# alpc91/SGRL

Hardware: AMD Instinct MI355X
Metric: env-steps/sec (whole node) + SET-actor fwd us/step, 3d_walker mix @8192 envs/GPU (higher is better)
Workload: dtype f64 (dynamics) / f32 (SET actor, obs); 1 GPU; 3D_Walker++ 8 variants x 1024 envs per GPU (config 3), random U(-1,1) actions, auto-reset, SET actor forward on every step, random-init weights; envs_per_gpu=8192, obs_max_len=287, action_max_len=21, replay_gather=none (single rank)

## Files before the change

include/sgrl.h:

```cpp
#ifndef SGRL_H
#define SGRL_H

#include <stdint.h>

#ifdef __cplusplus
extern "C" {
#endif

typedef struct sgrl_engine sgrl_engine;

enum {
  SGRL_OK = 0,
  SGRL_ERR_ARG = -1,
  SGRL_ERR_MODEL = -2,
  SGRL_ERR_HIP = -3,
  SGRL_ERR_LIMIT = -4
};

int sgrl_engine_create(int n_morph, const int32_t* const* ib, const int32_t* ib_len, const double* const* fb,
                       const int32_t* fb_len, const int32_t* morph_count, int obs_max_len, int action_max_len,
                       uint64_t seed, uint32_t env_id_base, int max_episode_steps, sgrl_engine** out);
void sgrl_engine_destroy(sgrl_engine* e);

int sgrl_num_envs(const sgrl_engine* e);
// ... 10 lines not shown
int sgrl_step(sgrl_engine* e, const float* actions, float* obs, float* reward, uint8_t* done, float* dist,
              uint8_t* truncated, double* obs64, double* reward64, int auto_reset, void* stream);

int sgrl_get_records(sgrl_engine* e, double* rec, int32_t* cnt);
int sgrl_set_records(sgrl_engine* e, const double* rec, const int32_t* cnt);
int sgrl_refresh(sgrl_engine* e, float* obs, double* obs64, void* stream);

int sgrl_time_steps(sgrl_engine* e, const float* actions, float* obs, float* reward, uint8_t* done, int reps,
                    void* stream, float* ms_out);

int sgrl_pack_transitions(const float* obs, int ld_obs, const float* action, int ld_act, const float* next_obs, int ld_next,
                          const float* reward, const float* done_f32, const uint8_t* done_u8, const uint8_t* store,
                          const int64_t* morph_id, float* block, int n_env, int obs_len, int act_len, void* stream);

int sgrl_round_record(const float* reward, const uint8_t* done, uint8_t* done_list, int64_t* ep_steps, float* ep_reward, float* reward_buf,
                      uint8_t* store, float* done_bool, int32_t* all_done, int n_env, int max_episode_steps, void* stream);

int sgrl_round_record_all(const float* reward, const uint8_t* done, uint8_t* done_list, int64_t* ep_steps, float* ep_reward, float* reward_buf,
                          int64_t* cur_steps, uint8_t* store, float* done_bool, int32_t* all_done, int32_t* was_complete, int n_env,
                          int max_episode_steps, void* stream);

typedef struct sgrl_ring {
  float* obs; float* action; float* next_obs; float* reward; float* done;
  int32_t obs_dim, act_dim;
} sgrl_ring;
int sgrl_ingest_rows(const float* block, int n_rows, int obs_len, int act_len, const int64_t* slot, const sgrl_ring* rings,
                     int n_rings, void* stream);
int64_t sgrl_ingest_ws_words(int n_rows);
int sgrl_ingest_block(const float* block, int n_rows, int obs_len, int act_len, const sgrl_ring* rings, int n_rings, int64_t* pos,
                      const int64_t* cap, int64_t* pending, int64_t* slot_ws, void* stream);

#define SGRL_DEBUG_CHOL_LD 352
int sgrl_debug_chol_solve(int flags, const int32_t* n, const double* C, const double* rhs, double* C_out, double* x_out, int32_t* ok);

const char* sgrl_last_error(void);
const char* sgrl_version(void);

#ifdef __cplusplus
}
#endif
#endif
```

sgrl_amd/_lib.py:

```python
import ctypes
import os
import subprocess

_HERE = os.path.dirname(os.path.abspath(__file__))
LIB_PATH = os.environ.get("SGRL_HIP_LIB", os.path.join(_HERE, "libsgrl_hip.so"))
CSRC = os.path.join(_HERE, "csrc")
SOURCES = ["engine.hip", "set_actor.hip", "train_gemm.hip", "render.hip", "swat_actor.hip", "smp_actor.hip", "replay_sample.hip", "eval_record.hip", "explore_actions.hip", "scene.hip", "mlp_actor.hip", "mlp_train.hip", "mlp_optim.hip", "mlp_batch.hip", "smp_train.hip", "td3_loss.hip", "dropout.hip"]

_lib = None

_i32p = ctypes.POINTER(ctypes.c_int32)
_f64p = ctypes.POINTER(ctypes.c_double)


class SgrlError(RuntimeError):
    pass


HDR_DIM_FIELDS = (1, 2, 3, 4, 5, 6, 7, 8, 9, 16, 18)
LIGHT_NV = 12
ITAB_GLOBAL = set(x for x in os.environ.get("SGRL_BUILD_ITAB_GLOBAL", "humanoid").split(",") if x and x != "none")
PAIR_NV = {"walker": 15, "hopper": 15}


# ... 118 lines not shown
    L.sgrl_time_steps.argtypes = [vp, vp, vp, vp, vp, ctypes.c_int, vp, ctypes.POINTER(ctypes.c_float)]
    ci = ctypes.c_int
    L.sgrl_pack_transitions.argtypes = [vp, ci, vp, ci, vp, ci, vp, vp, vp, vp, vp, vp, ci, ci, ci, vp]
    L.sgrl_ingest_rows.argtypes = [vp, ci, ci, ci, vp, vp, ci, vp]
    L.sgrl_ingest_block.argtypes = [vp, ci, ci, ci, vp, ci, vp, vp, vp, vp, vp]
    L.sgrl_reset_where.argtypes = [vp, vp, vp, vp, vp]
    L.sgrl_round_record.argtypes = [vp, vp, vp, vp, vp, vp, vp, vp, vp, ci, ci, vp]
    L.sgrl_round_record_all.argtypes = [vp, vp, vp, vp, vp, vp, vp, vp, vp, vp, vp, ci, ci, vp]
    L.sgrl_ingest_ws_words.argtypes = [ci]
    L.sgrl_ingest_ws_words.restype = ctypes.c_int64
    _lib = L
    return L


EXPLORE_GAUSS, EXPLORE_UNIFORM = 0, 1


def bind_explore(L):
    if getattr(L, "_explore_bound", False):
        return L
    vp, ci, cf = ctypes.c_void_p, ctypes.c_int, ctypes.c_float
    L.sgrl_explore_actions.argtypes = [vp, ci, vp, ci, vp, ci, ci, ctypes.c_int64, ctypes.c_uint64, ctypes.c_uint64, ci, cf, cf, cf, vp]
    L.sgrl_explore_actions.restype = ci
    L.sgrl_explore_actions_launches.argtypes = []
    L.sgrl_explore_actions_launches.restype = ci
    L.sgrl_explore_last_error.argtypes = []
    L.sgrl_explore_last_error.restype = ctypes.c_char_p
    L._explore_bound = True
    return L


EXPORTS = ["sgrl_engine_create", "sgrl_engine_destroy", "sgrl_num_envs", "sgrl_record_stride", "sgrl_lds_bytes", "sgrl_launch_groups", "sgrl_fixed_dim_groups", "sgrl_paired_envs",
           "sgrl_reset", "sgrl_reset_where", "sgrl_step", "sgrl_get_records", "sgrl_set_records", "sgrl_refresh", "sgrl_time_steps", "sgrl_pack_transitions", "sgrl_round_record", "sgrl_round_record_all", "sgrl_ingest_rows", "sgrl_ingest_block", "sgrl_ingest_ws_words",
           "sgrl_debug_chol_solve", "sgrl_last_error", "sgrl_version"]


def check(rc, what):
    if rc != 0:
        raise SgrlError("%s failed (%d): %s" % (what, rc, lib().sgrl_last_error().decode()))
```

sgrl_amd/csrc/engine.hip:

```cpp
#include <hip/hip_runtime.h>

#include <algorithm>
#include <cmath>
#include <cstdio>
#include <cstdlib>
#include <cstring>
#include <string>
#include <vector>

#include "engine_kernel.h"
#include "stream_pick.h"

namespace {

thread_local std::string g_err;

int fail(int code, const std::string& msg) {
  g_err = msg;
  return code;
}
#define HIP_TRY(expr)                                                                              \
  do {                                                                                             \
    hipError_t _e = (expr);                                                                        \
    if (_e != hipSuccess)                                                                          \
// ... 1 lines not shown
  } while (0)

using namespace sgrl_engine_dev;

__global__ __launch_bounds__(64) __attribute__((amdgpu_waves_per_eu(2, 2))) void k_env_step(BatchArgs a, StepOut out) {
  env_step_wave<DimsAny, sgrl::HipWave>(a, out, __builtin_amdgcn_readfirstlane(a.block_env[blockIdx.x]));
}

constexpr int kLightNv = 15;
constexpr int kLightPerCu = 12;
__global__ __launch_bounds__(64) __attribute__((amdgpu_waves_per_eu(3, 3))) void k_env_step_light(BatchArgs a, StepOut out) {
  env_step_wave<DimsAny, sgrl::HipWaveT<kLightNv>>(a, out, __builtin_amdgcn_readfirstlane(a.block_env[blockIdx.x]));
}

__global__ __launch_bounds__(64) void k_env_reset(BatchArgs a, StepOut out) {
  const int env = __builtin_amdgcn_readfirstlane(a.block_env[blockIdx.x]);
  if (out.done && !__builtin_amdgcn_readfirstlane((int)out.done[env])) return;
  SgrlModelView m; sgrl::Layout o; double* S; int32_t* I;
  setup<DimsAny>(a, env, &m, &o, &S, &I);
  sgrl::HipWave w;
  const sgrl::StepIO io = make_io(a, out, env);
  sgrl::env_reset(w, m, o, S, I, io, true);
}

__global__ __launch_bounds__(64) void k_env_refresh(BatchArgs a, StepOut out) {
  const int env = __builtin_amdgcn_readfirstlane(a.block_env[blockIdx.x]);
  SgrlModelView m; sgrl::Layout o; double* S; int32_t* I;
  setup<DimsAny>(a, env, &m, &o, &S, &I);
  sgrl::HipWave w;
  const sgrl::StepIO io = make_io(a, out, env);
  sgrl::env_refresh(w, m, o, S, I, io);
}

template <class Wv>
__device__ __forceinline__ void debug_chol_solve(Wv& w, int n, double* C, double* x, double* wv, bool inverse, int32_t* ok) {
  bool done;
  if (!inverse) {
    done = w.chol_solve_packed(n, C, x, sgrl::kMinVal);
  } else {
    done = w.chol_inv_packed(n, C, sgrl::kMinVal);
    if (done) {
      w.lanes(n, [&](int i) {
        double z = 0;
        for (int c = 0; c <= i; c++) z += C[i * (i + 1) / 2 + c] * x[c];
        wv[i] = z;
      });
      w.lanes(n, [&](int k) {
        double s = 0;
        for (int i = k; i < n; i++) s += C[i * (i + 1) / 2 + k] * wv[i];
        x[k] = s;
      });
    }
  }
  if (w.lane == 0) *ok = done ? 1 : 0;
}
__global__ __launch_bounds__(64) void k_debug_chol_solve(int flags, const int32_t* n, const double* C, const double* rhs, double* C_out,
                                                         double* x_out, int32_t* ok) {
  constexpr int LD = SGRL_DEBUG_CHOL_LD;
  __shared__ double sC[2 * LD], sx[64], swv[64];
  const int t = threadIdx.x;
  for (int i = t; i < 2 * LD; i += 64) sC[i] = C[i];
  sx[t] = rhs[t];
  swv[t] = 0.0;
  __syncthreads();
  if (flags & 1) {
    sgrl::HalfWaveT<15, sgrl::HipHalfPrim<sgrl::DimsAny>> w;
    const int h = w.half;
    debug_chol_solve(w, n[h], sC + h * LD, sx + h * 32, swv + h * 32, (flags & 2) != 0, ok + h);
  } else {
    sgrl::HipWave w;
    debug_chol_solve(w, n[0], sC, sx, swv, (flags & 2) != 0, ok);
  }
  __syncthreads();
  for (int i = t; i < 2 * LD; i += 64) C_out[i] = sC[i];
  x_out[t] = sx[t];
}

typedef int (*SpecLaunch)(int, int, void*, const void*, const void*);
struct SpecFamily { int waves; int n; SpecLaunch launch; int itab_global; };
struct SpecMember { int family, slot; int dims[12]; };
}
#ifndef SGRL_NO_SPECS
#define SGRL_FAMILY(id, waves, n, itab) extern "C" int sgrl_spec_launch_##id(int, int, void*, const void*, const void*);
#define SGRL_MEMBER(...)
#include "spec_table.inc"
#undef SGRL_FAMILY
#undef SGRL_MEMBER
namespace {
const SpecFamily kFamilies[] = {
#define SGRL_FAMILY(id, waves, n, itab) {waves, n, sgrl_spec_launch_##id, itab},
#define SGRL_MEMBER(...)
#include "spec_table.inc"
#undef SGRL_FAMILY
#undef SGRL_MEMBER
};
const SpecMember kMembers[] = {
#define SGRL_FAMILY(id, waves, n, itab)
#define SGRL_MEMBER(fam, slot, ...) {fam, slot, {__VA_ARGS__}},
#include "spec_table.inc"
#undef SGRL_FAMILY
#undef SGRL_MEMBER
};
constexpr int kNumMembers = (int)(sizeof(kMembers) / sizeof(kMembers[0]));
}
// ... 264 lines not shown
  const int k = r < n_rows ? w.key[r] : -1;
  keys[t] = k;
  {
    const int ring = t & 31, grp = t >> 5;
    int p = 0;
    for (int g = grp; g < c; g += 8) p += w.chunk_hist[g * kIngestMaxRings + ring];
    part[grp][ring] = p;
  }
  __syncthreads();
  long long sl = -1;
  if (k >= 0) {
    int rank = 0;
#pragma unroll
    for (int g = 0; g < 8; g++) rank += part[g][k];
    for (int j = 0; j < t; j++) rank += keys[j] == k ? 1 : 0;
    sl = (w.base[k] + rank) % cap[k];
  }
  if (r < n_rows) slot[r] = sl;
}

extern "C" {

const char* sgrl_last_error(void) { return g_err.c_str(); }
const char* sgrl_version(void) { return "sgrl-hip 0.2.0 (gfx950)"; }
#ifdef SGRL_PHASE_PROF
int sgrl_phase_prof(unsigned long long* host, int n_env, int reset) {
  if (hipDeviceSynchronize() != hipSuccess) return -1;
  if (host && hipMemcpyFromSymbol(host, HIP_SYMBOL(sgrl_engine_dev::g_phase_prof), sizeof(unsigned long long) * 16 * (size_t)n_env) != hipSuccess) return -2;
  if (reset) { static unsigned long long z[16 * 65536]; if (hipMemcpyToSymbol(HIP_SYMBOL(sgrl_engine_dev::g_phase_prof), z, sizeof(z)) != hipSuccess) return -3; }
  return 0;
}
#endif

int sgrl_debug_chol_solve(int flags, const int32_t* n, const double* C, const double* rhs, double* C_out, double* x_out, int32_t* ok) {
  constexpr int LD = SGRL_DEBUG_CHOL_LD;
  if (!n || !C || !rhs || !C_out || !x_out || !ok) return fail(SGRL_ERR_ARG, "sgrl_debug_chol_solve: null pointer");
  for (int p = 0; p < ((flags & 1) ? 2 : 1); p++)
    if (n[p] < 0 || n[p] * (n[p] + 1) / 2 > LD) return fail(SGRL_ERR_ARG, "sgrl_debug_chol_solve: n out of range");
  const size_t bytes = sizeof(double) * (4 * LD + 128) + sizeof(int32_t) * 4;
  char* d = nullptr;
  HIP_TRY(hipMalloc((void**)&d, bytes));
  double* dC = (double*)d; double* dCo = dC + 2 * LD; double* dr = dCo + 2 * LD; double* dx = dr + 64;
  int32_t* dn = (int32_t*)(dx + 64); int32_t* dok = dn + 2;
  const int32_t n2[2] = {n[0], (flags & 1) ? n[1] : 0};
  hipError_t e = hipMemset(d, 0, bytes);
  if (e == hipSuccess) e = hipMemcpy(dC, C, sizeof(double) * 2 * LD, hipMemcpyHostToDevice);
  if (e == hipSuccess) e = hipMemcpy(dr, rhs, sizeof(double) * 64, hipMemcpyHostToDevice);
  if (e == hipSuccess) e = hipMemcpy(dn, n2, sizeof(n2), hipMemcpyHostToDevice);
  if (e == hipSuccess) {
    k_debug_chol_solve<<<1, 64>>>(flags, dn, dC, dr, dCo, dx, dok);
    e = hipGetLastError();
  }
  if (e == hipSuccess) e = hipDeviceSynchronize();
  if (e == hipSuccess) e = hipMemcpy(C_out, dCo, sizeof(double) * 2 * LD, hipMemcpyDeviceToHost);
  if (e == hipSuccess) e = hipMemcpy(x_out, dx, sizeof(double) * 64, hipMemcpyDeviceToHost);
  if (e == hipSuccess) e = hipMemcpy(ok, dok, sizeof(int32_t) * 2, hipMemcpyDeviceToHost);
  (void)hipFree(d);
  if (e != hipSuccess) return fail(SGRL_ERR_HIP, std::string("sgrl_debug_chol_solve: ") + hipGetErrorString(e));
  return SGRL_OK;
}

void sgrl_engine_destroy(sgrl_engine* e) {
  if (!e) return;
  for (auto p : e->d_ib) if (p) (void)hipFree(p);
  for (auto p : e->d_fb) if (p) (void)hipFree(p);
  if (e->d_morphs) (void)hipFree(e->d_morphs);
  if (e->d_env_morph) (void)hipFree(e->d_env_morph);
  if (e->d_block_env) (void)hipFree(e->d_block_env);
  if (e->d_step_env) (void)hipFree(e->d_step_env);
  if (e->d_step_mate) (void)hipFree(e->d_step_mate);
  if (e->d_rec) (void)hipFree(e->d_rec);
  if (e->d_cnt) (void)hipFree(e->d_cnt);
  if (e->d_scratch) (void)hipFree(e->d_scratch);
  if (e->d_cam_dist) (void)hipFree(e->d_cam_dist);
  for (auto& g : e->groups) { if (g.stream) (void)hipStreamDestroy(g.stream); if (g.done) (void)hipEventDestroy(g.done); }
  if (e->fork) (void)hipEventDestroy(e->fork);
  delete e;
}

int sgrl_engine_create(int n_morph, const int32_t* const* ib, const int32_t* ib_len, const double* const* fb,
                       const int32_t* fb_len, const int32_t* morph_count, int obs_max_len, int action_max_len,
                       uint64_t seed, uint32_t env_id_base, int max_episode_steps, sgrl_engine** out) {
  if (!out) return fail(SGRL_ERR_ARG, "out is null");
  *out = nullptr;
  if (n_morph <= 0 || !ib || !ib_len || !fb || !fb_len || !morph_count) return fail(SGRL_ERR_ARG, "null or empty morphology list");
  int ndev = 0;
  (void)hipGetLastError();
  const hipError_t dev_err = hipGetDeviceCount(&ndev);
  if (dev_err != hipSuccess || ndev == 0)
    return fail(SGRL_ERR_HIP, std::string("no HIP device visible: libsgrl_hip.so needs an MI355X (there is no CPU fallback) [") +
                                  hipGetErrorString(dev_err) + ", " + std::to_string(ndev) + " devices]");
  sgrl_engine* e = new sgrl_engine();
// ... 407 lines not shown
```

sgrl_amd/csrc/wave_half.h:

```cpp
#pragma once
#include <stdint.h>

#include "step_body.h"

namespace sgrl {

template <int NVCAP, class P>
struct HalfWaveT : P {
  static_assert(NVCAP <= 16, "the register solvers of a half wave keep one matrix row per lane of ONE 16-lane DPP row");
  using P::lane;
  static constexpr int kLanes = 32;

  template <class F> SGRL_DEV void lanes(int n, F f) {
    for (int i = lane; i < n; i += kLanes) f(i);
    P::sync();
  }
  template <class F> SGRL_DEV void lanes_from(int lo, int hi, F f) {
    for (int i = lo + lane; i < hi; i += kLanes) f(i);
    P::sync();
  }
  template <class F> SGRL_DEV double sum(int n, F f) {
    double p = 0.0;
    for (int i = lane; i < n; i += kLanes) p += f(i);
    return P::half_sum(p);
  }
  template <class F> SGRL_DEV double maxabs(int n, F f) {
    double p = 0.0;
    for (int i = lane; i < n; i += kLanes) p = fmax(p, fabs(f(i)));
    return P::half_max(p);
  }
  template <class F> SGRL_DEV uint64_t ballot(int n, F f) {
    uint64_t m = P::half_ballot(lane < n ? (bool)f(lane) : false);
    if (n > kLanes) m |= (uint64_t)P::half_ballot(lane + kLanes < n ? (bool)f(lane + kLanes) : false) << 32;
    return m;
  }

  template <int NMAX>
  SGRL_DEV void chol_inv_reg(int n, double* Pm, double minval) {
    const bool act = lane < n;
    const int li = act ? lane : 0;
    double* rowp = Pm + li * (li + 1) / 2;
    double a[NMAX + 1];
#pragma unroll
    for (int k = 0; k < NMAX; k++) a[k + 1] = rowp[k < li ? k : li];
    double mydj = 0.0;
#pragma unroll
    for (int j = 0; j < NMAX; j++) {
      if (j < n) {
        const double c = a[j + 1];
        double pj = P::bcast16(c, j);
        pj = pj < minval ? minval : pj;
        const double dj = inv_sqrt(pj);
        const double l = c * dj;
        mydj = lane == j ? dj : mydj;
        const double lm = lane > j ? l * dj : 0.0;
        a[j] = lane == j ? 1.0 : 0.0;
#pragma unroll
        for (int c2 = 0; c2 <= j; c2++) a[c2] -= lm * P::bcast16(a[c2], j);
#pragma unroll
        for (int k = j + 1; k < NMAX; k++) a[k + 1] -= l * P::bcast16(l, k);
      }
    }
    if (act) {
#pragma unroll
      for (int k = NMAX - 1; k >= 0; k--) rowp[k < li ? k : li] = a[k] * mydj;
    }
    P::sync();
  }
  SGRL_DEV bool chol_inv_packed(int n, double* Pm, double minval) {
    if (NVCAP >= 9 && n <= 9) chol_inv_reg<9>(n, Pm, minval);
    else if (NVCAP >= 12 && n <= 12) chol_inv_reg<12>(n, Pm, minval);
    else if (NVCAP >= 15 && n <= 15) chol_inv_reg<15>(n, Pm, minval);
    else return false;
    return true;
  }

  template <int NMAX>
  SGRL_DEV void chol_solve_reg(int n, double* Pm, double* x, double minval) {
    const bool act = lane < n;
    const int li = act ? lane : 0;
    double* rowp = Pm + li * (li + 1) / 2;
    double a[NMAX];
#pragma unroll
    for (int k = 0; k < NMAX; k++) a[k] = rowp[k < li ? k : li];
    double r = x[li];
#pragma unroll
    for (int j = 0; j < NMAX; j++) {
      if (j < n) {
        const double c = a[j];
        double pj = P::bcast16(c, j);
        pj = pj < minval ? minval : pj;
        const double dj = inv_sqrt(pj);
        const double l = c * dj;
        const double lb = lane > j ? l : 0.0;
        const double zj = P::bcast16(r, j) * dj;
        r = lane == j ? zj * dj : r - lb * zj;
        a[j] = lb * dj;
#pragma unroll
        for (int k = j + 1; k < NMAX; k++) a[k] -= l * P::bcast16(l, k);
      }
    }
    if (act) {
#pragma unroll
      for (int k = NMAX - 1; k >= 0; k--) rowp[k < li ? k : li] = a[k];
    }
    P::sync();
    const int nl = n > 0 ? n - 1 : 0;
#pragma unroll
    for (int j = 1; j < NMAX; j++) {
      const int jj = j < nl ? j : nl;
      a[j] = Pm[jj * (jj + 1) / 2 + (lane < jj ? lane : jj)];
    }
#pragma unroll
    for (int j = NMAX - 1; j >= 1; j--) {
      if (j < n) r -= a[j] * P::bcast16(r, j);
    }
    if (act) x[lane] = r;
    P::sync();
  }
  SGRL_DEV bool chol_solve_packed(int n, double* Pm, double* x, double minval) {
    if (n <= 3) chol_solve_reg<3>(n, Pm, x, minval);
    else if (n <= 6) chol_solve_reg<6>(n, Pm, x, minval);
    else if (NVCAP >= 9 && n <= 9) chol_solve_reg<9>(n, Pm, x, minval);
    else if (NVCAP >= 12 && n <= 12) chol_solve_reg<12>(n, Pm, x, minval);
    else if (NVCAP >= 15 && n <= 15) chol_solve_reg<15>(n, Pm, x, minval);
    else return false;
    return true;
  }

  template <int NMAX>
  SGRL_DEV void trmm_rows_reg(int nrhs, int n, const double* T, double* Y, int ldy) {
    constexpr int NH = (NMAX + 1) / 2;
    const int h = lane & 1;
    for (int r0 = 0; r0 < nrhs; r0 += kLanes / 2) {
      const int r = r0 + (lane >> 1);
      const bool act = r < nrhs;
      double* y = Y + (act ? r : nrhs - 1) * ldy;
      double jr[NH];
#pragma unroll
      for (int u = 0; u < NH; u++) {
        const int c = 2 * u + h;
        const double v = y[c < n ? c : n - 1];
        jr[u] = c < n ? v : 0.0;
      }
#pragma unroll
      for (int d = (NMAX - 1) | 1; d >= 1; d -= 2) {
        if (d - 1 < n) {
          const double* Td = T + d * (d + 1) / 2 + h;
          const double* Te = T + (d - 1) * d / 2 + h;
          double s0 = 0.0, s1 = 0.0, e0 = 0.0, e1 = 0.0;
#pragma unroll
          for (int u = 0; u < NH; u++) {
            if (2 * u + 1 <= d) {
              const double td = Td[2 * u], te = Te[2 * u];
              const double tem = (2 * u + 1 <= d - 1) ? te : (h == 0 ? te : 0.0);
              if (u & 1) { s1 += td * jr[u]; e1 += tem * jr[u]; } else { s0 += td * jr[u]; e0 += tem * jr[u]; }
            }
          }
// ... 88 lines not shown
```

sgrl_amd/csrc/wave_hip.h:

```cpp
#pragma once
#include <hip/hip_runtime.h>

#include "../../include/sgrl_model.h"

namespace sgrl {

template <int CTRL>
__device__ __forceinline__ double dpp_move(double x) {
  int lo = __double2loint(x), hi = __double2hiint(x);
  lo = __builtin_amdgcn_update_dpp(0, lo, CTRL, 0xF, 0xF, false);
  hi = __builtin_amdgcn_update_dpp(0, hi, CTRL, 0xF, 0xF, false);
  return __hiloint2double(hi, lo);
}
__device__ __forceinline__ double read_lane(double x, int l) {
  const int lo = __builtin_amdgcn_readlane(__double2loint(x), l);
  const int hi = __builtin_amdgcn_readlane(__double2hiint(x), l);
  return __hiloint2double(hi, lo);
}
__device__ __forceinline__ double wave_sum(double x) {
  x += dpp_move<0xB1>(x);
  x += dpp_move<0x4E>(x);
  x += dpp_move<0x141>(x);
  x += dpp_move<0x140>(x);
  return (read_lane(x, 0) + read_lane(x, 16)) + (read_lane(x, 32) + read_lane(x, 48));
}
__device__ __forceinline__ double wave_max(double x) {
  x = fmax(x, dpp_move<0xB1>(x));
  x = fmax(x, dpp_move<0x4E>(x));
  x = fmax(x, dpp_move<0x141>(x));
  x = fmax(x, dpp_move<0x140>(x));
  return fmax(fmax(read_lane(x, 0), read_lane(x, 16)), fmax(read_lane(x, 32), read_lane(x, 48)));
}

struct DimsAny {
  static constexpr bool kFixed = false;
  static constexpr bool kPair = false;
  __device__ static __forceinline__ void apply(int32_t*) {}
  template <class M> __device__ static __forceinline__ int hdr_const(const M& m, int idx) { return m.hdr[idx]; }
};
struct DimsAny;
template <int NB, int NJ, int NQ, int NV, int NU, int NG, int NP, int INTEG, int FSKIP, int MAXROWS, int SOLVER, int PAIR = 0>
struct DimsFixed {
  static constexpr bool kFixed = true;
  static constexpr int kNv = NV;
  static constexpr bool kPair = PAIR != 0;
  static_assert(PAIR == 0 || NV <= 15, "two-environments-per-wavefront instances are built for at most 15 dofs");
  __device__ static __forceinline__ void apply(int32_t* hdr) {
    hdr[SGRL_H_NBODY] = NB; hdr[SGRL_H_NJNT] = NJ; hdr[SGRL_H_NQ] = NQ; hdr[SGRL_H_NV] = NV; hdr[SGRL_H_NU] = NU;
    hdr[SGRL_H_NGEOM] = NG; hdr[SGRL_H_NPAIR] = NP; hdr[SGRL_H_INTEGRATOR] = INTEG; hdr[SGRL_H_FRAME_SKIP] = FSKIP;
    hdr[SGRL_H_MAX_ROWS] = MAXROWS; hdr[SGRL_H_SOLVER] = SOLVER;
// ... 88 lines not shown
    const int n = __builtin_amdgcn_readfirstlane(n_in), nv = __builtin_amdgcn_readfirstlane(nv_in);
    const int iters = __builtin_amdgcn_readfirstlane(iters_in);
    const bool dofl = lane < nv;
    const int dl = dofl ? lane : 0;
    double vv = 0.0;
    for (int r = 0; r < n; r++) {
      const double fr = f[r];
      const double y = Y[r * ldy + dl];
      if (dofl) vv += y * fr;
    }
    int it = 0;
    for (; it < iters; it++) {
      double change = 0.0;
      double yn = Y[dl], bn = b[0], Rn = R[0], in_ = idg[0], fn_ = f[0];
      for (int r = 0; r < n; r++) {
        const double y = dofl ? yn : 0.0, br = bn, Rr = Rn, ir = in_, fr = fn_;
        if (r + 1 < n) { yn = Y[(r + 1) * ldy + dl]; bn = b[r + 1]; Rn = R[r + 1]; in_ = idg[r + 1]; fn_ = f[r + 1]; }
        const double dot = wave_sum(y * vv);
        const double res = br + Rr * fr + dot;
        double fnew = fr - res * ir;
        fnew = fnew < 0.0 ? 0.0 : fnew;
        const double df = fnew - fr;
        vv += y * df;
        if (lane == 0) f[r] = fnew;
        change = fmax(change, fabs(df) / ir);
      }
      __syncthreads();
      if (change < thresh) { it++; break; }
    }
    if (dofl) v[lane] = vv;
    __syncthreads();
    return it;
  }
  template <int NMAX>
  __device__ __forceinline__ void chol_inv_reg(int n, double* P, double minval) {
    const bool act = lane < n;
    const int li = act ? lane : 0;
    double* rowp = P + li * (li + 1) / 2;
    double a[NMAX + 1];
#pragma unroll
    for (int k = 0; k < NMAX; k++) a[k + 1] = rowp[k < li ? k : li];
    double mydj = 0.0;
#pragma unroll
    for (int j = 0; j < NMAX; j++) {
      if (j < n) {
        const double c = a[j + 1];
        double pj = read_lane(c, j);
        pj = pj < minval ? minval : pj;
        const double dj = rsqrt(pj);
        const double l = c * dj;
        mydj = lane == j ? dj : mydj;
        const double lm = lane > j ? l * dj : 0.0;
        a[j] = lane == j ? 1.0 : 0.0;
#pragma unroll
        for (int c2 = 0; c2 <= j; c2++) a[c2] -= lm * read_lane(a[c2], j);
#pragma unroll
        for (int k = j + 1; k < NMAX; k++) a[k + 1] -= l * read_lane(l, k);
      }
    }
    if (act) {
#pragma unroll
      for (int k = NMAX - 1; k >= 0; k--) rowp[k < li ? k : li] = a[k] * mydj;
    }
    __syncthreads();
  }
  __device__ __forceinline__ bool chol_inv_packed(int n_in, double* P, double minval) {
    const int n = __builtin_amdgcn_readfirstlane(n_in);
    if (NVCAP >= 9 && n <= 9) chol_inv_reg<9>(n, P, minval);
    else if (NVCAP >= 12 && n <= 12) chol_inv_reg<12>(n, P, minval);
    else if (NVCAP >= 15 && n <= 15) chol_inv_reg<15>(n, P, minval);
    else if (NVCAP >= 18 && n <= 18) chol_inv_reg<18>(n, P, minval);
    else if (NVCAP >= 21 && n <= 21) chol_inv_reg<21>(n, P, minval);
    else if (NVCAP >= 24 && n <= 24) chol_inv_reg<24>(n, P, minval);
    else return false;
    return true;
  }
  template <int NMAX>
  __device__ __forceinline__ void chol_solve_reg(int n, double* P, double* x, double minval) {
    const bool act = lane < n;
    const int li = act ? lane : 0;
    double* rowp = P + li * (li + 1) / 2;
    double a[NMAX];
#pragma unroll
    for (int k = 0; k < NMAX; k++) a[k] = rowp[k < li ? k : li];
    double r = x[li];
#pragma unroll
    for (int j = 0; j < NMAX; j++) {
      if (j < n) {
        const double c = a[j];
        double pj = read_lane(c, j);
        pj = pj < minval ? minval : pj;
        const double dj = rsqrt(pj);
        const double l = c * dj;
        const double lb = lane > j ? l : 0.0;
        const double zj = read_lane(r, j) * dj;
        r = lane == j ? zj * dj : r - lb * zj;
        a[j] = lb * dj;
#pragma unroll
        for (int k = j + 1; k < NMAX; k++) a[k] -= l * read_lane(l, k);
      }
    }
    if (act) {
#pragma unroll
      for (int k = NMAX - 1; k >= 0; k--) rowp[k < li ? k : li] = a[k];
    }
    __syncthreads();
    const int nl = n > 0 ? n - 1 : 0;
#pragma unroll
    for (int j = 1; j < NMAX; j++) {
      const int jj = j < nl ? j : nl;
      a[j] = P[jj * (jj + 1) / 2 + (lane < jj ? lane : jj)];
    }
#pragma unroll
    for (int j = NMAX - 1; j >= 1; j--) {
      if (j < n) r -= a[j] * read_lane(r, j);
    }
    if (act) x[lane] = r;
    __syncthreads();
  }
  __device__ __forceinline__ bool chol_solve_packed(int n_in, double* P, double* x, double minval) {
    const int n = __builtin_amdgcn_readfirstlane(n_in);
    if (n <= 3) chol_solve_reg<3>(n, P, x, minval);
    else if (n <= 6) chol_solve_reg<6>(n, P, x, minval);
    else if (NVCAP >= 9 && n <= 9) chol_solve_reg<9>(n, P, x, minval);
    else if (NVCAP >= 12 && n <= 12) chol_solve_reg<12>(n, P, x, minval);
    else if (NVCAP >= 15 && n <= 15) chol_solve_reg<15>(n, P, x, minval);
    else if (NVCAP >= 18 && n <= 18) chol_solve_reg<18>(n, P, x, minval);
    else if (NVCAP >= 21 && n <= 21) chol_solve_reg<21>(n, P, x, minval);
    else if (NVCAP >= 24 && n <= 24) chol_solve_reg<24>(n, P, x, minval);
    else return false;
    return true;
  }
  template <int NMAX>
  __device__ __forceinline__ void trmm_rows_reg(int nrhs, int n, const double* T, double* Y, int ldy) {
    constexpr int NH = (NMAX + 1) / 2;
    const int h = lane & 1;
    for (int r0 = 0; r0 < nrhs; r0 += 32) {
      const int r = r0 + (lane >> 1);
      const bool act = r < nrhs;
      double* y = Y + (act ? r : nrhs - 1) * ldy;
      double jr[NH];
#pragma unroll
      for (int u = 0; u < NH; u++) {
        const int c = 2 * u + h;
        const double v = y[c < n ? c : n - 1];
        jr[u] = c < n ? v : 0.0;
      }
#pragma unroll
      for (int d = (NMAX - 1) | 1; d >= 1; d -= 2) {
        if (d - 1 < n) {
          const double* Td = T + d * (d + 1) / 2 + h;
          const double* Te = T + (d - 1) * d / 2 + h;
          double s0 = 0.0, s1 = 0.0, e0 = 0.0, e1 = 0.0;
#pragma unroll
          for (int u = 0; u < NH; u++) {
            if (2 * u + 1 <= d) {
              const double td = Td[2 * u], te = Te[2 * u];
              const double tem = (2 * u + 1 <= d - 1) ? te : (h == 0 ? te : 0.0);
              if (u & 1) { s1 += td * jr[u]; e1 += tem * jr[u]; } else { s0 += td * jr[u]; e0 += tem * jr[u]; }
            }
          }
          double sd = s0 + s1, se = e0 + e1;
// ... 179 lines not shown
    return wave_max(p);
  }
};
using HipWave = HipWaveT<24>;

template <class D>
struct HipHalfPrim {
  static constexpr bool kFixedDims = D::kFixed;
  template <class M> __device__ static __forceinline__ int hdr_const(const M& m, int idx) { return D::hdr_const(m, idx); }
  int lane;
  int half;
  __device__ __forceinline__ HipHalfPrim() : lane(threadIdx.x & 31), half((threadIdx.x >> 5) & 1) {}
#ifdef SGRL_PHASE_PROF
  __device__ __forceinline__ void tick(int) {}
#endif
  __device__ __forceinline__ void fence_lane() { asm volatile("" : "+v"(lane)); }
  template <class T> __device__ __forceinline__ T fenced(T v) {
    int t = __builtin_amdgcn_readfirstlane((int)(unsigned)(__UINTPTR_TYPE__)v);
    asm volatile("" : "+s"(t));
    return (T)(__UINTPTR_TYPE__)(unsigned)t;
  }
  __device__ static __forceinline__ void sync() { __syncthreads(); }
  __device__ static __forceinline__ double bcast16(double x, int j) {
    switch (j) {
      case 0: return dpp_move<0x150>(x);   case 1: return dpp_move<0x151>(x);   case 2: return dpp_move<0x152>(x);
      case 3: return dpp_move<0x153>(x);   case 4: return dpp_move<0x154>(x);   case 5: return dpp_move<0x155>(x);
      case 6: return dpp_move<0x156>(x);   case 7: return dpp_move<0x157>(x);   case 8: return dpp_move<0x158>(x);
      case 9: return dpp_move<0x159>(x);   case 10: return dpp_move<0x15A>(x);  case 11: return dpp_move<0x15B>(x);
      case 12: return dpp_move<0x15C>(x);  case 13: return dpp_move<0x15D>(x);  case 14: return dpp_move<0x15E>(x);
      default: return dpp_move<0x15F>(x);
    }
  }
  __device__ static __forceinline__ double xor1(double x) { return dpp_move<0xB1>(x); }
  __device__ static __forceinline__ void rows_of_half(double x, double* even, double* odd) {
    const unsigned lo = (unsigned)__double2loint(x), hi = (unsigned)__double2hiint(x);
    const auto l = __builtin_amdgcn_permlane16_swap(lo, lo, false, false);
    const auto h = __builtin_amdgcn_permlane16_swap(hi, hi, false, false);
    *even = __hiloint2double((int)h[0], (int)l[0]);
    *odd = __hiloint2double((int)h[1], (int)l[1]);
  }
  __device__ static __forceinline__ double half_sum(double x) {
    x += dpp_move<0xB1>(x);
    x += dpp_move<0x4E>(x);
    x += dpp_move<0x141>(x);
    x += dpp_move<0x140>(x);
    double e, o;
    rows_of_half(x, &e, &o);
    return e + o;
  }
  __device__ static __forceinline__ double half_max(double x) {
    x = fmax(x, dpp_move<0xB1>(x));
    x = fmax(x, dpp_move<0x4E>(x));
    x = fmax(x, dpp_move<0x141>(x));
    x = fmax(x, dpp_move<0x140>(x));
    double e, o;
    rows_of_half(x, &e, &o);
    return fmax(e, o);
  }
  __device__ __forceinline__ uint32_t half_ballot(bool p) const {
    const uint64_t b = (uint64_t)__ballot(p);
    return half ? (uint32_t)(b >> 32) : (uint32_t)b;
  }
};

}
```

Baseline: 2.083 million env-steps/s.

## Fuse Cholesky broadcast-multiply-subtract into DPP row_newbcast fmac inline asm

New measurement: 2.127 million env-steps/s (median of 6 runs). 2.2% higher.

```diff
diff --git a/include/sgrl.h b/include/sgrl.h
--- a/include/sgrl.h
+++ b/include/sgrl.h
@@ -66,6 +66,8 @@
 
 #define SGRL_DEBUG_CHOL_LD 352
 int sgrl_debug_chol_solve(int flags, const int32_t* n, const double* C, const double* rhs, double* C_out, double* x_out, int32_t* ok);
+int sgrl_debug_chol_solve_form(int form, int flags, const int32_t* n, const double* C, const double* rhs, double* C_out, double* x_out, int32_t* ok);
+int sgrl_debug_chol_inv(int form, int policy, const int32_t* n, const double* C, double* C_out, int32_t* ok);
 
 const char* sgrl_last_error(void);
 const char* sgrl_version(void);
diff --git a/sgrl_amd/_lib.py b/sgrl_amd/_lib.py
--- a/sgrl_amd/_lib.py
+++ b/sgrl_amd/_lib.py
@@ -174,7 +174,7 @@
 
 EXPORTS = ["sgrl_engine_create", "sgrl_engine_destroy", "sgrl_num_envs", "sgrl_record_stride", "sgrl_lds_bytes", "sgrl_launch_groups", "sgrl_fixed_dim_groups", "sgrl_paired_envs",
            "sgrl_reset", "sgrl_reset_where", "sgrl_step", "sgrl_get_records", "sgrl_set_records", "sgrl_refresh", "sgrl_time_steps", "sgrl_pack_transitions", "sgrl_round_record", "sgrl_round_record_all", "sgrl_ingest_rows", "sgrl_ingest_block", "sgrl_ingest_ws_words",
-           "sgrl_debug_chol_solve", "sgrl_last_error", "sgrl_version"]
+           "sgrl_debug_chol_solve", "sgrl_debug_chol_solve_form", "sgrl_debug_chol_inv", "sgrl_last_error", "sgrl_version"]
 
 
 def check(rc, what):
diff --git a/sgrl_amd/csrc/engine.hip b/sgrl_amd/csrc/engine.hip
--- a/sgrl_amd/csrc/engine.hip
+++ b/sgrl_amd/csrc/engine.hip
@@ -57,13 +57,15 @@
   sgrl::env_refresh(w, m, o, S, I, io);
 }
 
-template <class Wv>
-__device__ __forceinline__ void debug_chol_solve(Wv& w, int n, double* C, double* x, double* wv, bool inverse, int32_t* ok) {
+template <int FORM, class Wv>
+__device__ __forceinline__ void debug_chol_solve(Wv& w, int n, double* C, double* x, double* wv, bool inverse, bool inverse_only, int32_t* ok) {
   bool done;
-  if (!inverse) {
-    done = w.chol_solve_packed(n, C, x, sgrl::kMinVal);
+  if (inverse_only) {
+    done = w.template chol_inv_packed<FORM>(n, C, sgrl::kMinVal);
+  } else if (!inverse) {
+    done = w.template chol_solve_packed<FORM>(n, C, x, sgrl::kMinVal);
   } else {
-    done = w.chol_inv_packed(n, C, sgrl::kMinVal);
+    done = w.template chol_inv_packed<FORM>(n, C, sgrl::kMinVal);
     if (done) {
       w.lanes(n, [&](int i) {
         double z = 0;
@@ -88,13 +90,16 @@
   sx[t] = rhs[t];
   swv[t] = 0.0;
   __syncthreads();
+  const bool inv = (flags & 2) != 0, inv_only = (flags & 8) != 0;
   if (flags & 1) {
     sgrl::HalfWaveT<15, sgrl::HipHalfPrim<sgrl::DimsAny>> w;
     const int h = w.half;
-    debug_chol_solve(w, n[h], sC + h * LD, sx + h * 32, swv + h * 32, (flags & 2) != 0, ok + h);
+    if (flags & 4) debug_chol_solve<0>(w, n[h], sC + h * LD, sx + h * 32, swv + h * 32, inv, inv_only, ok + h);
+    else debug_chol_solve<1>(w, n[h], sC + h * LD, sx + h * 32, swv + h * 32, inv, inv_only, ok + h);
   } else {
     sgrl::HipWave w;
-    debug_chol_solve(w, n[0], sC, sx, swv, (flags & 2) != 0, ok);
+    if (flags & 4) debug_chol_solve<0>(w, n[0], sC, sx, swv, inv, inv_only, ok);
+    else debug_chol_solve<1>(w, n[0], sC, sx, swv, inv, inv_only, ok);
   }
   __syncthreads();
   for (int i = t; i < 2 * LD; i += 64) C_out[i] = sC[i];
@@ -425,23 +430,24 @@
 }
 #endif
 
-int sgrl_debug_chol_solve(int flags, const int32_t* n, const double* C, const double* rhs, double* C_out, double* x_out, int32_t* ok) {
+static int debug_chol_run(const char* who, int kflags, const int32_t* n, const double* C, const double* rhs, double* C_out, double* x_out, int32_t* ok) {
   constexpr int LD = SGRL_DEBUG_CHOL_LD;
-  if (!n || !C || !rhs || !C_out || !x_out || !ok) return fail(SGRL_ERR_ARG, "sgrl_debug_chol_solve: null pointer");
-  for (int p = 0; p < ((flags & 1) ? 2 : 1); p++)
-    if (n[p] < 0 || n[p] * (n[p] + 1) / 2 > LD) return fail(SGRL_ERR_ARG, "sgrl_debug_chol_solve: n out of range");
+  const std::string name(who);
+  if (!n || !C || !rhs || !C_out || !x_out || !ok) return fail(SGRL_ERR_ARG, name + ": null pointer");
+  for (int p = 0; p < ((kflags & 1) ? 2 : 1); p++)
+    if (n[p] < 0 || n[p] * (n[p] + 1) / 2 > LD) return fail(SGRL_ERR_ARG, name + ": n out of range");
   const size_t bytes = sizeof(double) * (4 * LD + 128) + sizeof(int32_t) * 4;
   char* d = nullptr;
   HIP_TRY(hipMalloc((void**)&d, bytes));
   double* dC = (double*)d; double* dCo = dC + 2 * LD; double* dr = dCo + 2 * LD; double* dx = dr + 64;
   int32_t* dn = (int32_t*)(dx + 64); int32_t* dok = dn + 2;
-  const int32_t n2[2] = {n[0], (flags & 1) ? n[1] : 0};
+  const int32_t n2[2] = {n[0], (kflags & 1) ? n[1] : 0};
   hipError_t e = hipMemset(d, 0, bytes);
   if (e == hipSuccess) e = hipMemcpy(dC, C, sizeof(double) * 2 * LD, hipMemcpyHostToDevice);
   if (e == hipSuccess) e = hipMemcpy(dr, rhs, sizeof(double) * 64, hipMemcpyHostToDevice);
   if (e == hipSuccess) e = hipMemcpy(dn, n2, sizeof(n2), hipMemcpyHostToDevice);
   if (e == hipSuccess) {
-    k_debug_chol_solve<<<1, 64>>>(flags, dn, dC, dr, dCo, dx, dok);
+    k_debug_chol_solve<<<1, 64>>>(kflags, dn, dC, dr, dCo, dx, dok);
     e = hipGetLastError();
   }
   if (e == hipSuccess) e = hipDeviceSynchronize();
@@ -449,8 +455,22 @@
   if (e == hipSuccess) e = hipMemcpy(x_out, dx, sizeof(double) * 64, hipMemcpyDeviceToHost);
   if (e == hipSuccess) e = hipMemcpy(ok, dok, sizeof(int32_t) * 2, hipMemcpyDeviceToHost);
   (void)hipFree(d);
-  if (e != hipSuccess) return fail(SGRL_ERR_HIP, std::string("sgrl_debug_chol_solve: ") + hipGetErrorString(e));
-  return SGRL_OK;
+  if (e != hipSuccess) return fail(SGRL_ERR_HIP, name + ": " + hipGetErrorString(e));
+  return SGRL_OK;
+}
+
+int sgrl_debug_chol_solve(int flags, const int32_t* n, const double* C, const double* rhs, double* C_out, double* x_out, int32_t* ok) {
+  return debug_chol_run("sgrl_debug_chol_solve", flags & 3, n, C, rhs, C_out, x_out, ok);
+}
+int sgrl_debug_chol_solve_form(int form, int flags, const int32_t* n, const double* C, const double* rhs, double* C_out, double* x_out, int32_t* ok) {
+  if (form != 0 && form != 1) return fail(SGRL_ERR_ARG, "sgrl_debug_chol_solve_form: form must be 0 or 1");
+  return debug_chol_run("sgrl_debug_chol_solve_form", (flags & 3) | (form ? 0 : 4), n, C, rhs, C_out, x_out, ok);
+}
+int sgrl_debug_chol_inv(int form, int policy, const int32_t* n, const double* C, double* C_out, int32_t* ok) {
+  if (form != 0 && form != 1) return fail(SGRL_ERR_ARG, "sgrl_debug_chol_inv: form must be 0 or 1");
+  const double rhs[64] = {0};
+  double x_out[64];
+  return debug_chol_run("sgrl_debug_chol_inv", (policy & 1) | 8 | (form ? 0 : 4), n, C, rhs, C_out, x_out, ok);
 }
 
 void sgrl_engine_destroy(sgrl_engine* e) {
diff --git a/sgrl_amd/csrc/wave_half.h b/sgrl_amd/csrc/wave_half.h
--- a/sgrl_amd/csrc/wave_half.h
+++ b/sgrl_amd/csrc/wave_half.h
@@ -4,6 +4,11 @@
 #include "step_body.h"
 
 namespace sgrl {
+
+template <class P, class = void>
+struct HasFnmaBcast { static constexpr int value = 0; };
+template <class P>
+struct HasFnmaBcast<P, decltype((void)P::template fnma_run<1, 0>(ref_of<double*>(), 0.0, 0.0))> { static constexpr int value = 1; };
 
 template <int NVCAP, class P>
 struct HalfWaveT : P {
@@ -35,7 +40,25 @@
     return m;
   }
 
-  template <int NMAX>
+  template <int NMAX, int J>
+  SGRL_DEV void chol_inv_pivots_fnma(int n, double* a, double& mydj, double minval) {
+    if constexpr (J < NMAX) {
+      if (J < n) {
+        const double c = a[J + 1];
+        double pj = P::template bcast16c<J>(c);
+        pj = pj < minval ? minval : pj;
+        const double dj = inv_sqrt(pj);
+        const double l = c * dj;
+        mydj = lane == J ? dj : mydj;
+        const double lm = lane > J ? l * dj : 0.0;
+        a[J] = lane == J ? 1.0 : 0.0;
+        P::template fnma_self<J + 1, J>(a, lm);
+        P::template fnma_run<NMAX - 1 - J, J + 1>(a + J + 2, l, l);
+      }
+      chol_inv_pivots_fnma<NMAX, J + 1>(n, a, mydj, minval);
+    }
+  }
+  template <int NMAX, int FORM = HasFnmaBcast<P>::value>
   SGRL_DEV void chol_inv_reg(int n, double* Pm, double minval) {
     const bool act = lane < n;
     const int li = act ? lane : 0;
@@ -44,6 +67,8 @@
 #pragma unroll
     for (int k = 0; k < NMAX; k++) a[k + 1] = rowp[k < li ? k : li];
     double mydj = 0.0;
+    if constexpr (FORM == 1) chol_inv_pivots_fnma<NMAX, 0>(n, a, mydj, minval);
+    else
 #pragma unroll
     for (int j = 0; j < NMAX; j++) {
       if (j < n) {
@@ -67,15 +92,41 @@
     }
     P::sync();
   }
+  template <int FORM = HasFnmaBcast<P>::value>
   SGRL_DEV bool chol_inv_packed(int n, double* Pm, double minval) {
-    if (NVCAP >= 9 && n <= 9) chol_inv_reg<9>(n, Pm, minval);
-    else if (NVCAP >= 12 && n <= 12) chol_inv_reg<12>(n, Pm, minval);
-    else if (NVCAP >= 15 && n <= 15) chol_inv_reg<15>(n, Pm, minval);
+    if (NVCAP >= 9 && n <= 9) chol_inv_reg<9, FORM>(n, Pm, minval);
+    else if (NVCAP >= 12 && n <= 12) chol_inv_reg<12, FORM>(n, Pm, minval);
+    else if (NVCAP >= 15 && n <= 15) chol_inv_reg<15, FORM>(n, Pm, minval);
     else return false;
     return true;
   }
 
-  template <int NMAX>
+  template <int NMAX, int J>
+  SGRL_DEV void chol_solve_pivots_fnma(int n, double* a, double& r, double minval) {
+    if constexpr (J < NMAX) {
+      if (J < n) {
+        const double c = a[J];
+        double pj = P::template bcast16c<J>(c);
+        pj = pj < minval ? minval : pj;
+        const double dj = inv_sqrt(pj);
+        const double l = c * dj;
+        const double lb = lane > J ? l : 0.0;
+        const double zj = P::template bcast16c<J>(r) * dj;
+        r = lane == J ? zj * dj : r - lb * zj;
+        a[J] = lb * dj;
+        P::template fnma_run<NMAX - 1 - J, J + 1>(a + J + 1, l, l);
+      }
+      chol_solve_pivots_fnma<NMAX, J + 1>(n, a, r, minval);
+    }
+  }
+  template <int J>
+  SGRL_DEV void chol_solve_back_fnma(int n, double* a, double& r) {
+    if constexpr (J >= 1) {
+      if (J < n) P::template fnma_self<1, J>(&r, a[J]);
+      chol_solve_back_fnma<J - 1>(n, a, r);
+    }
+  }
+  template <int NMAX, int FORM = HasFnmaBcast<P>::value>
   SGRL_DEV void chol_solve_reg(int n, double* Pm, double* x, double minval) {
     const bool act = lane < n;
     const int li = act ? lane : 0;
@@ -84,6 +135,8 @@
 #pragma unroll
     for (int k = 0; k < NMAX; k++) a[k] = rowp[k < li ? k : li];
     double r = x[li];
+    if constexpr (FORM == 1) chol_solve_pivots_fnma<NMAX, 0>(n, a, r, minval);
+    else
 #pragma unroll
     for (int j = 0; j < NMAX; j++) {
       if (j < n) {
@@ -111,6 +164,8 @@
       const int jj = j < nl ? j : nl;
       a[j] = Pm[jj * (jj + 1) / 2 + (lane < jj ? lane : jj)];
     }
+    if constexpr (FORM == 1) chol_solve_back_fnma<NMAX - 1>(n, a, r);
+    else
 #pragma unroll
     for (int j = NMAX - 1; j >= 1; j--) {
       if (j < n) r -= a[j] * P::bcast16(r, j);
@@ -118,12 +173,13 @@
     if (act) x[lane] = r;
     P::sync();
   }
+  template <int FORM = HasFnmaBcast<P>::value>
   SGRL_DEV bool chol_solve_packed(int n, double* Pm, double* x, double minval) {
-    if (n <= 3) chol_solve_reg<3>(n, Pm, x, minval);
-    else if (n <= 6) chol_solve_reg<6>(n, Pm, x, minval);
-    else if (NVCAP >= 9 && n <= 9) chol_solve_reg<9>(n, Pm, x, minval);
-    else if (NVCAP >= 12 && n <= 12) chol_solve_reg<12>(n, Pm, x, minval);
-    else if (NVCAP >= 15 && n <= 15) chol_solve_reg<15>(n, Pm, x, minval);
+    if (n <= 3) chol_solve_reg<3, FORM>(n, Pm, x, minval);
+    else if (n <= 6) chol_solve_reg<6, FORM>(n, Pm, x, minval);
+    else if (NVCAP >= 9 && n <= 9) chol_solve_reg<9, FORM>(n, Pm, x, minval);
+    else if (NVCAP >= 12 && n <= 12) chol_solve_reg<12, FORM>(n, Pm, x, minval);
+    else if (NVCAP >= 15 && n <= 15) chol_solve_reg<15, FORM>(n, Pm, x, minval);
     else return false;
     return true;
   }
diff --git a/sgrl_amd/csrc/wave_hip.h b/sgrl_amd/csrc/wave_hip.h
--- a/sgrl_amd/csrc/wave_hip.h
+++ b/sgrl_amd/csrc/wave_hip.h
@@ -16,6 +16,66 @@
   const int lo = __builtin_amdgcn_readlane(__double2loint(x), l);
   const int hi = __builtin_amdgcn_readlane(__double2hiint(x), l);
   return __hiloint2double(hi, lo);
+}
+#define SGRL_REP1(M, S) M(0)
+#define SGRL_REP2(M, S) SGRL_REP1(M, S) S() M(1)
+#define SGRL_REP3(M, S) SGRL_REP2(M, S) S() M(2)
+#define SGRL_REP4(M, S) SGRL_REP3(M, S) S() M(3)
+#define SGRL_REP5(M, S) SGRL_REP4(M, S) S() M(4)
+#define SGRL_REP6(M, S) SGRL_REP5(M, S) S() M(5)
+#define SGRL_REP7(M, S) SGRL_REP6(M, S) S() M(6)
+#define SGRL_REP8(M, S) SGRL_REP7(M, S) S() M(7)
+#define SGRL_REP9(M, S) SGRL_REP8(M, S) S() M(8)
+#define SGRL_REP10(M, S) SGRL_REP9(M, S) S() M(9)
+#define SGRL_REP11(M, S) SGRL_REP10(M, S) S() M(10)
+#define SGRL_REP12(M, S) SGRL_REP11(M, S) S() M(11)
+#define SGRL_REP13(M, S) SGRL_REP12(M, S) S() M(12)
+#define SGRL_REP14(M, S) SGRL_REP13(M, S) S() M(13)
+#define SGRL_REP15(M, S) SGRL_REP14(M, S) S() M(14)
+#define SGRL_REP16(M, S) SGRL_REP15(M, S) S() M(15)
+#define SGRL_REP17(M, S) SGRL_REP16(M, S) S() M(16)
+#define SGRL_REP18(M, S) SGRL_REP17(M, S) S() M(17)
+#define SGRL_REP19(M, S) SGRL_REP18(M, S) S() M(18)
+#define SGRL_REP20(M, S) SGRL_REP19(M, S) S() M(19)
+#define SGRL_REP21(M, S) SGRL_REP20(M, S) S() M(20)
+#define SGRL_REP22(M, S) SGRL_REP21(M, S) S() M(21)
+#define SGRL_REP23(M, S) SGRL_REP22(M, S) S() M(22)
+#define SGRL_REP24(M, S) SGRL_REP23(M, S) S() M(23)
+#define SGRL_SEP_NONE()
+#define SGRL_SEP_COMMA() ,
+#define SGRL_DPP_ACC(i) "+v"(p[i])
+#define SGRL_DPP_RUN(i) "v_fmac_f64_dpp %" #i ", %[s], -%[m] row_newbcast:%c[j]+" #i " row_mask:0xf bank_mask:0xf\n\t"
+#define SGRL_DPP_SELF(i) "v_fmac_f64_dpp %" #i ", %" #i ", -%[m] row_newbcast:%c[j] row_mask:0xf bank_mask:0xf\n\t"
+#define SGRL_DPP_CASE_RUN(n) \
+  else if constexpr (N == n) asm volatile("s_nop 4\n\t" SGRL_REP##n(SGRL_DPP_RUN, SGRL_SEP_NONE) "s_nop 1" : SGRL_REP##n(SGRL_DPP_ACC, SGRL_SEP_COMMA) : [s] "v"(src), [m] "v"(mul), [j] "i"(J0));
+#define SGRL_DPP_CASE_SELF(n) \
+  else if constexpr (N == n) asm volatile("s_nop 4\n\t" SGRL_REP##n(SGRL_DPP_SELF, SGRL_SEP_NONE) "s_nop 1" : SGRL_REP##n(SGRL_DPP_ACC, SGRL_SEP_COMMA) : [m] "v"(mul), [j] "i"(J));
+#define SGRL_DPP_CASES(C) C(1) C(2) C(3) C(4) C(5) C(6) C(7) C(8) C(9) C(10) C(11) C(12) C(13) C(14) C(15) C(16) C(17) C(18) C(19) C(20) C(21) C(22) C(23) C(24)
+template <int N, int J0>
+__device__ __forceinline__ void fnma_bcast16_run(double* p, double src, double mul) {
+  static_assert(N <= 24 && J0 >= 0 && J0 + N <= 16, "one asm statement: at most 24 accumulators, lanes of one 16-lane row");
+  if constexpr (N <= 0) {}
+  SGRL_DPP_CASES(SGRL_DPP_CASE_RUN)
+}
+template <int N, int J>
+__device__ __forceinline__ void fnma_bcast16_self(double* p, double mul) {
+  static_assert(N <= 24 && J >= 0 && J < 16, "one asm statement: at most 24 accumulators, a lane of the 16-lane row");
+  if constexpr (N <= 0) {}
+  SGRL_DPP_CASES(SGRL_DPP_CASE_SELF)
+}
+template <int J>
+__device__ __forceinline__ void fnma_bcast16(double& acc, double src, double mul) { fnma_bcast16_run<1, J>(&acc, src, mul); }
+template <int J>
+__device__ __forceinline__ double bcast16_b64(double x) {
+  static_assert(J >= 0 && J < 16, "a lane of the 16-lane row");
+  return __builtin_amdgcn_update_dpp(0.0, x, 0x150 + J, 0xF, 0xF, false);
+}
+__device__ __forceinline__ void rows_of_half(double x, double* even, double* odd) {
+  const unsigned lo = (unsigned)__double2loint(x), hi = (unsigned)__double2hiint(x);
+  const auto l = __builtin_amdgcn_permlane16_swap(lo, lo, false, false);
+  const auto h = __builtin_amdgcn_permlane16_swap(hi, hi, false, false);
+  *even = __hiloint2double((int)h[0], (int)l[0]);
+  *odd = __hiloint2double((int)h[1], (int)l[1]);
 }
 __device__ __forceinline__ double wave_sum(double x) {
   x += dpp_move<0xB1>(x);
@@ -170,7 +230,45 @@
     __syncthreads();
     return it;
   }
-  template <int NMAX>
+  template <int NMAX, int J>
+  __device__ __forceinline__ void chol_inv_pivots_dpp(int n, double* a, double& mydj, double minval) {
+    if constexpr (J < NMAX) {
+      if (J < n) {
+        const double c = a[J + 1];
+        double pj;
+        if constexpr (NMAX <= 16) pj = bcast16_b64<J>(c); else pj = read_lane(c, J);
+        pj = pj < minval ? minval : pj;
+        const double dj = rsqrt(pj);
+        const double l = c * dj;
+        mydj = lane == J ? dj : mydj;
+        const double lm = lane > J ? l * dj : 0.0;
+        a[J] = lane == J ? 1.0 : 0.0;
+        if constexpr (NMAX <= 16) fnma_bcast16_self<J + 1, J>(a, lm);
+        else if constexpr (J >= 16) fnma_bcast16_self<J + 1, J - 16>(a, lm);
+        else {
+#pragma unroll
+          for (int c2 = 0; c2 <= J; c2++) a[c2] -= lm * read_lane(a[c2], J);
+        }
+        trailing_dpp<NMAX, J>(a + 1, l);
+      }
+      chol_inv_pivots_dpp<NMAX, J + 1>(n, a, mydj, minval);
+    }
+  }
+  template <int NMAX, int J>
+  __device__ __forceinline__ void trailing_dpp(double* a, double l) {
+    if constexpr (NMAX <= 16) {
+      fnma_bcast16_run<NMAX - 1 - J, J + 1>(a + J + 1, l, l);
+    } else {
+      constexpr int KB = J + 1 > 16 ? J + 1 : 16;
+      if constexpr (J + 1 < 16) {
+        double le, lo;
+        rows_of_half(l, &le, &lo);
+        fnma_bcast16_run<15 - J, J + 1>(a + J + 1, le, l);
+      }
+      fnma_bcast16_run<NMAX - KB, KB - 16>(a + KB, l, l);
+    }
+  }
+  template <int NMAX, int FORM = 1>
   __device__ __forceinline__ void chol_inv_reg(int n, double* P, double minval) {
     const bool act = lane < n;
     const int li = act ? lane : 0;
@@ -179,6 +277,8 @@
 #pragma unroll
     for (int k = 0; k < NMAX; k++) a[k + 1] = rowp[k < li ? k : li];
     double mydj = 0.0;
+    if constexpr (FORM == 1) chol_inv_pivots_dpp<NMAX, 0>(n, a, mydj, minval);
+    else
 #pragma unroll
     for (int j = 0; j < NMAX; j++) {
       if (j < n) {
@@ -202,18 +302,45 @@
     }
     __syncthreads();
   }
+  template <int FORM = 1>
   __device__ __forceinline__ bool chol_inv_packed(int n_in, double* P, double minval) {
     const int n = __builtin_amdgcn_readfirstlane(n_in);
-    if (NVCAP >= 9 && n <= 9) chol_inv_reg<9>(n, P, minval);
-    else if (NVCAP >= 12 && n <= 12) chol_inv_reg<12>(n, P, minval);
-    else if (NVCAP >= 15 && n <= 15) chol_inv_reg<15>(n, P, minval);
-    else if (NVCAP >= 18 && n <= 18) chol_inv_reg<18>(n, P, minval);
-    else if (NVCAP >= 21 && n <= 21) chol_inv_reg<21>(n, P, minval);
-    else if (NVCAP >= 24 && n <= 24) chol_inv_reg<24>(n, P, minval);
+    if (NVCAP >= 9 && n <= 9) chol_inv_reg<9, FORM>(n, P, minval);
+    else if (NVCAP >= 12 && n <= 12) chol_inv_reg<12, FORM>(n, P, minval);
+    else if (NVCAP >= 15 && n <= 15) chol_inv_reg<15, FORM>(n, P, minval);
+    else if (NVCAP >= 18 && n <= 18) chol_inv_reg<18, FORM>(n, P, minval);
+    else if (NVCAP >= 21 && n <= 21) chol_inv_reg<21, FORM>(n, P, minval);
+    else if (NVCAP >= 24 && n <= 24) chol_inv_reg<24, FORM>(n, P, minval);
     else return false;
     return true;
   }
-  template <int NMAX>
+  template <int NMAX, int J>
+  __device__ __forceinline__ void chol_solve_pivots_dpp(int n, double* a, double& r, double minval) {
+    if constexpr (J < NMAX) {
+      if (J < n) {
+        const double c = a[J];
+        double pj, rj;
+        if constexpr (NMAX <= 16) { pj = bcast16_b64<J>(c); rj = bcast16_b64<J>(r); } else { pj = read_lane(c, J); rj = read_lane(r, J); }
+        pj = pj < minval ? minval : pj;
+        const double dj = rsqrt(pj);
+        const double l = c * dj;
+        const double lb = lane > J ? l : 0.0;
+        const double zj = rj * dj;
+        r = lane == J ? zj * dj : r - lb * zj;
+        a[J] = lb * dj;
+        trailing_dpp<NMAX, J>(a, l);
+      }
+      chol_solve_pivots_dpp<NMAX, J + 1>(n, a, r, minval);
+    }
+  }
+  template <int J>
+  __device__ __forceinline__ void chol_solve_back_dpp(int n, double* a, double& r) {
+    if constexpr (J >= 1) {
+      if (J < n) fnma_bcast16_self<1, J>(&r, a[J]);
+      chol_solve_back_dpp<J - 1>(n, a, r);
+    }
+  }
+  template <int NMAX, int FORM = 1>
   __device__ __forceinline__ void chol_solve_reg(int n, double* P, double* x, double minval) {
     const bool act = lane < n;
     const int li = act ? lane : 0;
@@ -222,6 +349,8 @@
 #pragma unroll
     for (int k = 0; k < NMAX; k++) a[k] = rowp[k < li ? k : li];
     double r = x[li];
+    if constexpr (FORM == 1) chol_solve_pivots_dpp<NMAX, 0>(n, a, r, minval);
+    else
 #pragma unroll
     for (int j = 0; j < NMAX; j++) {
       if (j < n) {
@@ -249,6 +378,8 @@
       const int jj = j < nl ? j : nl;
       a[j] = P[jj * (jj + 1) / 2 + (lane < jj ? lane : jj)];
     }
+    if constexpr (FORM == 1 && NMAX <= 16) chol_solve_back_dpp<NMAX - 1>(n, a, r);
+    else
 #pragma unroll
     for (int j = NMAX - 1; j >= 1; j--) {
       if (j < n) r -= a[j] * read_lane(r, j);
@@ -256,16 +387,17 @@
     if (act) x[lane] = r;
     __syncthreads();
   }
+  template <int FORM = 1>
   __device__ __forceinline__ bool chol_solve_packed(int n_in, double* P, double* x, double minval) {
     const int n = __builtin_amdgcn_readfirstlane(n_in);
-    if (n <= 3) chol_solve_reg<3>(n, P, x, minval);
-    else if (n <= 6) chol_solve_reg<6>(n, P, x, minval);
-    else if (NVCAP >= 9 && n <= 9) chol_solve_reg<9>(n, P, x, minval);
-    else if (NVCAP >= 12 && n <= 12) chol_solve_reg<12>(n, P, x, minval);
-    else if (NVCAP >= 15 && n <= 15) chol_solve_reg<15>(n, P, x, minval);
-    else if (NVCAP >= 18 && n <= 18) chol_solve_reg<18>(n, P, x, minval);
-    else if (NVCAP >= 21 && n <= 21) chol_solve_reg<21>(n, P, x, minval);
-    else if (NVCAP >= 24 && n <= 24) chol_solve_reg<24>(n, P, x, minval);
+    if (n <= 3) chol_solve_reg<3, FORM>(n, P, x, minval);
+    else if (n <= 6) chol_solve_reg<6, FORM>(n, P, x, minval);
+    else if (NVCAP >= 9 && n <= 9) chol_solve_reg<9, FORM>(n, P, x, minval);
+    else if (NVCAP >= 12 && n <= 12) chol_solve_reg<12, FORM>(n, P, x, minval);
+    else if (NVCAP >= 15 && n <= 15) chol_solve_reg<15, FORM>(n, P, x, minval);
+    else if (NVCAP >= 18 && n <= 18) chol_solve_reg<18, FORM>(n, P, x, minval);
+    else if (NVCAP >= 21 && n <= 21) chol_solve_reg<21, FORM>(n, P, x, minval);
+    else if (NVCAP >= 24 && n <= 24) chol_solve_reg<24, FORM>(n, P, x, minval);
     else return false;
     return true;
   }
@@ -511,13 +643,10 @@
     }
   }
   __device__ static __forceinline__ double xor1(double x) { return dpp_move<0xB1>(x); }
-  __device__ static __forceinline__ void rows_of_half(double x, double* even, double* odd) {
-    const unsigned lo = (unsigned)__double2loint(x), hi = (unsigned)__double2hiint(x);
-    const auto l = __builtin_amdgcn_permlane16_swap(lo, lo, false, false);
-    const auto h = __builtin_amdgcn_permlane16_swap(hi, hi, false, false);
-    *even = __hiloint2double((int)h[0], (int)l[0]);
-    *odd = __hiloint2double((int)h[1], (int)l[1]);
-  }
+  __device__ static __forceinline__ void rows_of_half(double x, double* even, double* odd) { sgrl::rows_of_half(x, even, odd); }
+  template <int N, int J0> __device__ static __forceinline__ void fnma_run(double* p, double src, double mul) { fnma_bcast16_run<N, J0>(p, src, mul); }
+  template <int N, int J> __device__ static __forceinline__ void fnma_self(double* p, double mul) { fnma_bcast16_self<N, J>(p, mul); }
+  template <int J> __device__ static __forceinline__ double bcast16c(double x) { return bcast16_b64<J>(x); }
   __device__ static __forceinline__ double half_sum(double x) {
     x += dpp_move<0xB1>(x);
     x += dpp_move<0x4E>(x);
```
